# mitschabaude/montgomery

Hardware: AMD Instinct MI355X
Metric: BLS12-377 G1 MSM throughput (higher is better)
Workload: dtype u32

## Files before the change

### montgomery_amd/csrc/msm_sort.hip

```cpp
#include "msm_internal.h"

using namespace msm;
using namespace msmi;

namespace msmi {

uint64_t one_level_entry_limit(bool te) { return te ? 1ull << 22 : 1ull << 21; }

void sort_kernel_attributes() {
  HIPCHK(hipFuncSetAttribute((const void*)k_hist, hipFuncAttributeMaxDynamicSharedMemorySize, 128 * 1024));
  HIPCHK(hipFuncSetAttribute((const void*)k_scatter_lds, hipFuncAttributeMaxDynamicSharedMemorySize, 128 * 1024));
  HIPCHK(hipFuncSetAttribute((const void*)k_bin_split, hipFuncAttributeMaxDynamicSharedMemorySize, (int)bin_split_lds(1u << BS_MAX_AB)));
  HIPCHK(hipFuncSetAttribute((const void*)k_bin_pairs, hipFuncAttributeMaxDynamicSharedMemorySize, (int)bin_pairs_lds(1u << BS_MAX_FB)));
  HIPCHK(hipFuncSetAttribute((const void*)k_bin_slots, hipFuncAttributeMaxDynamicSharedMemorySize, (int)bin_slots_lds(1u << BS_MAX_FB)));
  const int dig_lds = 16 * (1 << BS_MAX_AB) * 4;
#define MSM_DIGITS_ATTR(ID, CV) HIPCHK(hipFuncSetAttribute((const void*)k_digits<CV>, hipFuncAttributeMaxDynamicSharedMemorySize, dig_lds));
  MSM_W_CURVES(MSM_DIGITS_ATTR)
#undef MSM_DIGITS_ATTR
  HIPCHK(hipFuncSetAttribute((const void*)te::k_te_digits, hipFuncAttributeMaxDynamicSharedMemorySize, dig_lds));
#define MSM_NARROW_ATTR(W)                                                                                                    \
  HIPCHK(hipFuncSetAttribute((const void*)k_digits_narrow<W>, hipFuncAttributeMaxDynamicSharedMemorySize, dig_lds));          \
  HIPCHK(hipFuncSetAttribute((const void*)k_te_digits_narrow<W>, hipFuncAttributeMaxDynamicSharedMemorySize, dig_lds));
  MSM_NARROW_WIDTHS(MSM_NARROW_ATTR)
#undef MSM_NARROW_ATTR
}

static void narrow_digits(msm_ctx* ctx, msm_ctx::Workspace& w, const uint32_t* d_scalars, uint64_t n, const Plan& pl, int k_lo, int kc_d,
                          bool bin_split, bool radix, uint32_t sortB, uint64_t pps, uint32_t hb, const WinSplit& ws) {
  hipStream_t s = w.stream;
  const bool te = ctx->is_te();
  const int W = pl.nar.width, per_lane = W == 1 ? 4 : W == 2 ? 2 : 1;
  uint32_t* dig = (uint32_t*)w.dig.p;
  uint32_t* err = (uint32_t*)ctx->errflag.p;
  const int fold = pl.fold ? 1 : 0;
  if (pl.batch) {
    if (bin_split || radix || k_lo != 0 || kc_d != pl.batch * pl.K || !pl.nar.nb) throw MsmFail{MSM_ERR_INTERNAL, "a batch group outside the one-level sort"};
    const uint32_t grid = (uint32_t)(((n + per_lane - 1) / per_lane + 255) / 256);
#define MSM_NARROW_LAUNCH_B(WW)                                                                                               \
  if (W == WW) {                                                                                                              \
    if (te) hipLaunchKernelGGL(k_te_digits_narrow_batch<WW>, dim3(grid), dim3(256), 0, s, dig, *pl.nar.nb, (uint32_t)pl.batch, \
                               (uint32_t)n, pl.c, pl.K, fold, pl.nar.fmt, err);                                               \
    else hipLaunchKernelGGL(k_digits_narrow_batch<WW>, dim3(grid), dim3(256), 0, s, dig, *pl.nar.nb, (uint32_t)pl.batch,      \
                            (uint32_t)n, pl.c, pl.K, fold, pl.nar.fmt, err);                                                  \
  }
    MSM_NARROW_WIDTHS(MSM_NARROW_LAUNCH_B)
#undef MSM_NARROW_LAUNCH_B
    return;
  }
  const uint32_t per = bin_split ? (uint32_t)pps : 256u * per_lane;
  const uint32_t grid = bin_split ? sortB : (uint32_t)((n + per - 1) / per);
  const uint32_t threads = bin_split ? 1024u : 256u;
  uint32_t* hist = bin_split ? (uint32_t*)w.block_hist.p : nullptr;
  const size_t lds = bin_split ? (size_t)kc_d * hb * 4 : 0;
  const uint64_t fbp = pack_fine_bits(ws);
#define MSM_NARROW_LAUNCH(WW)                                                                                                 \
  if (W == WW) {                                                                                                              \
    if (te) hipLaunchKernelGGL(k_te_digits_narrow<WW>, dim3(grid), dim3(threads), lds, s, dig, (const void*)d_scalars,        \
                               pl.nar.first, (uint32_t)n, pl.c, pl.K, k_lo, kc_d, fold, pl.nar.fmt, err, per, hist, hb, fbp); \
    else hipLaunchKernelGGL(k_digits_narrow<WW>, dim3(grid), dim3(threads), lds, s, dig, (const void*)d_scalars, pl.nar.first, \
                            (uint32_t)n, pl.c, pl.K, k_lo, kc_d, fold, pl.nar.fmt, err, per, hist, hb, fbp);                  \
  }
  MSM_NARROW_WIDTHS(MSM_NARROW_LAUNCH)
#undef MSM_NARROW_LAUNCH
}

void sort_window_group(msm_ctx* ctx, msm_ctx::Workspace& w, const uint32_t* d_scalars, uint64_t n, const Plan& pl, int k_lo, int k_hi,
                       GroupStats& st, SortOut& so, GroupDigits* share) {
  hipStream_t s = w.stream;
  const bool produce = share && share->produce;
  const bool consume = share && !share->produce && share->valid;
  const int kc_d = k_hi - k_lo;
  const uint32_t L = pl.L;
  const bool te = ctx->is_te();
  const uint64_t two_n_d = te ? n : 2 * n;
  const uint64_t n_entries = (uint64_t)kc_d * two_n_d;
  const int kc = pl.tables ? 1 : kc_d;
  const uint64_t two_n = pl.tables ? n_entries : two_n_d;
  const uint64_t nb = (uint64_t)kc * L;

  uint64_t mean = std::max<uint64_t>(1, two_n / (pl.fold ? L / 2 : L));
  uint64_t per_bucket_left = mean >= 512 ? 32 : (mean >= 128 || (mean >= 64 && pl.c >= 18 && !pl.tables)) ? 16 : 8;
  MSM_KNOB(per_bucket_left, "MSM_PBL", 1);
  uint32_t logG = 1;
  while (logG < 10 && (1ull << (logG + 1)) * per_bucket_left <= mean) logG++;

  if (!consume && !produce) ctx->ensure(w.dig, n_entries * 4);
  if (produce) {
    share->valid = false;
  } else {
  ctx->ensure(w.counts, nb * 4);
  ctx->ensure(w.cursor, (nb + 1) * 4);
  ctx->ensure(w.tail_off, (size_t)34 * (nb + 1) * 4);
  ctx->ensure(w.info, 64 * 4);
  }

  const int cbits = pl.L_log;
  const bool fits_lds = (size_t)L * 4 <= 128 * 1024;
  const bool want_radix = fits_lds && cbits > (int)RX_FINE_BITS && two_n >= one_level_entry_limit(te);
  const bool want_bins = !fits_lds || (pl.tables && two_n >= (1ull << 22));
  const bool bin_split = !fits_lds || want_bins;
  const bool radix = !bin_split && want_radix && cbits > (int)RX_FINE_BITS && cbits - (int)RX_FINE_BITS <= 8;
  WinSplit ws{};
  uint32_t hb = 1, nbmax = 1;
  if (bin_split) {
    if (kc > 16) throw MsmFail{MSM_ERR_INTERNAL, "more than 16 windows in a group of a window size above 16"};
    for (int kk = 0; kk < kc; kk++) {
      const bool top = (k_lo + kk) % pl.K == pl.K - 1;
      const int eff = pl.tables ? cbits : std::max(1, top ? std::min(cbits, pl.bits - (k_lo + kk) * pl.c) : std::min(cbits, pl.c - 1));
      const int ab_big = 10;
      const int abk = eff <= (int)ab_big ? eff : std::max((int)ab_big, eff - (int)BS_MAX_FB);
      if (abk > (int)BS_MAX_AB) throw MsmFail{MSM_ERR_INTERNAL, "window too wide for the bin split"};
      ws.ab[kk] = (uint8_t)abk;
      ws.fb[kk] = (uint8_t)(eff - abk);
      hb = std::max(hb, 1u << abk);
      nbmax = std::max(nbmax, 1u << (eff - abk));
    }
  } else if (radix) {
    if (kc > 16) throw MsmFail{MSM_ERR_INTERNAL, "more than 16 windows in a radix-split group"};
    for (int kk = 0; kk < kc; kk++) { ws.ab[kk] = (uint8_t)(cbits - (int)RX_FINE_BITS); ws.fb[kk] = (uint8_t)RX_FINE_BITS; }
  }
  const uint32_t Hn = radix ? 1u << (cbits - (int)RX_FINE_BITS) : 1u;
  const uint32_t V = (uint32_t)kc * (bin_split ? hb : Hn);
  uint32_t sortB = 1;
  uint64_t chunk = two_n, pps = n;
  if (bin_split) {
    const uint64_t mult = 4;
    sortB = (uint32_t)std::max<uint64_t>(1, std::min<uint64_t>((uint64_t)mult * ctx->n_cu, n / 4096));
    const uint64_t max_pps = (1ull << BS_SPAN_LOG) / (te ? 1 : 2);
    sortB = (uint32_t)std::max<uint64_t>(sortB, (n + max_pps - 1) / max_pps);
    pps = (n + sortB - 1) / sortB;
    chunk = (te ? 1 : 2) * pps;
    if (consume) {
      if (share->sortB != sortB || share->pps != pps || share->chunk != chunk || share->hb < hb)
        throw MsmFail{MSM_ERR_INTERNAL, "shared digits do not match the group's sort geometry"};
      hb = share->hb;
    } else {
      ctx->ensure(w.block_hist, (size_t)kc_d * sortB * hb * 4 + 64);
    }
  } else {
    const uint64_t mult = two_n >= (1ull << 27) ? 8 : two_n >= (1ull << 24) ? 4 : 2;
    uint64_t want = std::max<uint64_t>(1, (mult * ctx->n_cu + kc - 1) / kc);
    uint64_t maxb = std::max<uint64_t>(1, two_n / 8192);
    sortB = (uint32_t)std::min<uint64_t>(want, maxb);
    chunk = (two_n + sortB - 1) / sortB;
    if (!produce) ctx->ensure(w.block_hist, (size_t)kc * sortB * L * 4 + 64);
  }
  uint32_t* d_bin_start = nullptr;
  uint32_t *d_extra_first = nullptr, *d_mp_first = nullptr, *d_part_pair_off = nullptr;
  uint32_t part_len = 0, part_grid = 0;
  bool will_chunk = false;
  {
    const int chunk_rows_log = 23;
    const uint64_t table_rows = pl.tables ? (uint64_t)kc_d * n : n;
    const bool want_chunks = bin_split && !te && pl.c >= 18 && table_rows > (1ull << chunk_rows_log);
    will_chunk = bin_split && want_chunks && !te && logG >= 2;
  }
  if (produce && !bin_split) return;
  if (produce) ctx->ensure(w.dig, n_entries * 4);
  if (share && !share->produce && !bin_split) throw MsmFail{MSM_ERR_INTERNAL, "shared digits for a group that does not take the bin split"};
  const uint32_t* dig_p = consume ? share->dig + (uint64_t)(k_lo - share->k_lo) * two_n_d : (const uint32_t*)w.dig.p;
  uint32_t* hist_p = consume ? share->hist + (uint64_t)(k_lo - share->k_lo) * sortB * hb : (uint32_t*)w.block_hist.p;

  if (consume) HIPCHK(hipStreamWaitEvent(s, share->ready, 0));
  HIPCHK(hipEventRecord(w.ev[0], s));
  if (pl.nar.width) {
    if (!consume) narrow_digits(ctx, w, d_scalars, n, pl, k_lo, kc_d, bin_split, radix, sortB, pps, hb, ws);
  } else if (pl.batch) {
    if (bin_split || radix || k_lo != 0 || kc_d != pl.batch * pl.K) throw MsmFail{MSM_ERR_INTERNAL, "a batch group outside the one-level sort"};
    const uint32_t grid = (uint32_t)((n + 255) / 256);
    if (te)
      hipLaunchKernelGGL(te::k_te_digits_batch, dim3(grid), dim3(256), 0, s, (uint32_t*)w.dig.p, pl.batch_sc, (uint32_t)pl.batch,
                         (uint32_t)n, pl.c, pl.K, pl.strict ? 1 : 0, (uint32_t*)ctx->errflag.p);
    else
      W_LAUNCH(ctx, k_digits_batch, dim3(grid), dim3(256), 0, s, (uint32_t*)w.dig.p, pl.batch_sc, (uint32_t)pl.batch, (uint32_t)n, pl.c,
               pl.K, (pl.no_glv ? 0 : 1) | (pl.fold ? 2 : 0), pl.strict ? 1 : 0, (uint32_t*)ctx->errflag.p);
  } else if (!consume) {
    const uint32_t grid = bin_split ? sortB : (uint32_t)((n + 255) / 256);
    const uint32_t per = bin_split ? (uint32_t)pps : 256u;
    uint32_t* hist = bin_split ? (uint32_t*)w.block_hist.p : nullptr;
    const size_t lds = bin_split ? (size_t)kc_d * hb * 4 : 0;
    WinSplit ws_d = ws;
    if (pl.tables) for (int kk = 0; kk < 16; kk++) ws_d.fb[kk] = ws.fb[0];
    const uint32_t threads = bin_split ? 1024u : 256u;
    if (te)
      hipLaunchKernelGGL(te::k_te_digits, dim3(grid), dim3(threads), lds, s, (uint32_t*)w.dig.p, d_scalars, (uint32_t)n, pl.c, pl.K,
                         k_lo, kc_d, pl.strict ? 1 : 0, (uint32_t*)ctx->errflag.p, per, hist, hb, pack_fine_bits(ws_d), pl.b_lo, pl.b_n, pl.bt_lo, pl.bt_n);
    else
      W_LAUNCH(ctx, k_digits, dim3(grid), dim3(threads), lds, s, (uint32_t*)w.dig.p, d_scalars, (uint32_t)n, pl.c, pl.K, k_lo, kc_d,
                         (pl.no_glv ? 0 : 1) | (pl.fold ? 2 : 0), pl.strict ? 1 : 0, (uint32_t*)ctx->errflag.p, per, hist, hb, pack_fine_bits(ws_d), pl.b_lo, pl.b_n, pl.bt_lo, pl.bt_n);
  }
  if (produce) {
    share->k_lo = k_lo;
    share->dig = (const uint32_t*)w.dig.p;
    share->hist = (uint32_t*)w.block_hist.p;
    share->hb = hb;
    share->sortB = sortB;
    share->pps = pps;
    share->chunk = chunk;
    HIPCHK(hipEventRecord(share->ready, s));
    share->valid = true;
    return;
  }
  HIPCHK(hipEventRecord(w.ev[1], s));
  if (!bin_split) {
    hipLaunchKernelGGL(k_hist, dim3(sortB, kc), dim3(SORT_THREADS), (size_t)L * 4, s, (uint32_t*)w.block_hist.p,
                       (const uint32_t*)w.dig.p, two_n, chunk, L);
    hipLaunchKernelGGL(k_colscan, dim3((uint32_t)((nb + 255) / 256)), dim3(256), 0, s, (uint32_t*)w.block_hist.p,
                       (uint32_t*)w.counts.p, sortB, L, (uint32_t)kc);
  } else {
    ctx->ensure(w.part, ((size_t)2 * V + 2) * 4);
    uint32_t* d_bin_tot = (uint32_t*)w.part.p;
    d_bin_start = d_bin_tot + V;
    ctx->ensure(w.rec, n_entries * 8);
    hipLaunchKernelGGL(k_slice_scan, dim3((hb + 31) / 32, kc), dim3(1024), 0, s, hist_p, d_bin_tot,
                       pl.tables ? sortB * (uint32_t)kc_d : sortB, hb, (uint32_t)kc);
    part_len = (uint32_t)std::max<uint64_t>(1u << 16, ((2 * n_entries / V + BP_TILE - 1) / BP_TILE) * BP_TILE);
    part_grid = V + V / 2 + 1;
    ctx->ensure(w.parts, ((size_t)2 * (V + 1) + (V + 2)) * 4);
    d_extra_first = (uint32_t*)w.parts.p;
    d_mp_first = d_extra_first + (V + 1);
    d_part_pair_off = d_mp_first + (V + 1);
    PartTables ptab{d_extra_first, d_mp_first, d_part_pair_off, hb, part_len, {}};
    for (int kk = 0; kk < 16; kk++) ptab.fb[kk] = ws.fb[kk];
    hipLaunchKernelGGL(k_vscan, dim3(1), dim3(SCAN_THREADS), 0, s, d_bin_start, (const uint32_t*)d_bin_tot, V, (uint32_t*)w.info.p, ptab);
    const uint32_t per_block = (uint32_t)std::min<uint64_t>(std::min<uint64_t>(sortB, std::max<uint64_t>(1, (1ull << BS_SPAN_LOG) / chunk)),
                                                            std::max<uint64_t>(1, (2 * (uint64_t)BS_TILE + chunk - 1) / chunk));
    hipLaunchKernelGGL(k_bin_split, dim3((sortB + per_block - 1) / per_block, kc_d), dim3(BS_THREADS), bin_split_lds(hb), s, (uint2*)w.rec.p,
                       (const uint32_t*)d_bin_start, (const uint32_t*)hist_p, dig_p, two_n_d, chunk, hb, ws,
                       pl.tables ? 1u : 0u, sortB, per_block);
    bool spans_all = true;
    for (int kk = 0; kk < kc; kk++) spans_all &= (1u << ws.ab[kk]) == hb && (int)ws.ab[kk] + (int)ws.fb[kk] == cbits;
    if (!spans_all) HIPCHK(hipMemsetAsync(w.counts.p, 0, nb * 4, s));
    ctx->ensure(w.sub, (size_t)(V + 2) * nbmax * 4);
    hipLaunchKernelGGL(k_bin_count, dim3(part_grid), dim3(BC_THREADS), (size_t)nbmax * 4, s, (uint32_t*)w.counts.p, (const uint32_t*)d_bin_start,
                       (const uint2*)w.rec.p, hb, L, ws, (uint32_t*)w.info.p, V, (const uint32_t*)d_extra_first, (const uint32_t*)d_mp_first,
                       part_len, (uint32_t*)w.sub.p, nbmax);
    hipLaunchKernelGGL(k_part_scan, dim3(V), dim3(PSC_THREADS), 0, s, (uint32_t*)w.counts.p, (uint32_t*)w.sub.p, d_part_pair_off,
                       (const uint32_t*)d_extra_first, (const uint32_t*)d_mp_first, hb, L, nbmax, ws, (uint32_t*)w.info.p,
                       will_chunk ? 1u : 0u);
  }
  int RT = 0;
  uint64_t total_slots = 0;
  uint32_t max_bucket = 0;
  {
    if (!bin_split) {
      HIPCHK(hipMemsetAsync(w.info.p, 0, 64 * 4, s));
// ... 100 lines not shown
```

### montgomery_amd/csrc/msm_tree.hip

```cpp
#include "msm_internal.h"

using namespace msm;
using namespace msmi;

namespace msmi {

void accumulate_window_group(msm_ctx* ctx, msm_ctx::Workspace& w, const Plan& pl, int kc, uint64_t row_off, const SortOut& so,
                             GroupStats& st, TreeOut& to) {
  hipStream_t s = w.stream;
  const bool lone = pl.lone;
  const bool te = ctx->is_te();
  const uint32_t L = pl.L;
  const uint64_t nb = (uint64_t)kc * L;
  const size_t elem_bytes = te ? 128 : 96;
  const uint32_t logG = so.logG;
  const int RT = so.RT;
  const uint64_t total_slots = so.total_slots;
  const uint32_t max_bucket = so.max_bucket;
  const uint32_t* round1_slots = so.round1_slots;
  const uint32_t* round1_dest = so.round1_dest;
  const uint64_t rec_y_off = so.rec_y_off;
  const bool chunked = so.chunked;

  uint32_t FINISH_MAX = pl.c >= 18 ? 64 : 32;
  MSM_KNOB(FINISH_MAX, "MSM_FINISH_MAX", 1);
  uint32_t tail_min_pairs = pl.c >= 18 ? 1u << 23 : 1u << 21;
  MSM_KNOB(tail_min_pairs, "MSM_TAIL_MIN", 1);
  const bool use_finish = true;
  int r_stop = RT;
  if (use_finish) {
    uint32_t cap_elems = (max_bucket + (1u << logG) - 1) >> logG;
    r_stop = 0;
    while (r_stop < RT &&
           (((cap_elems + (1u << r_stop) - 1) >> r_stop) > FINISH_MAX || w.h_info[3 + r_stop + 1] >= tail_min_pairs))
      r_stop++;
  }
  uint64_t capA = 1, capB = 1;
  {
    int which = 0;
    uint64_t cnt = total_slots;
    for (uint32_t r = 1; r <= logG; r++) {
      cnt /= 2;
      if (r == 1 && chunked) continue;
      (which ? capB : capA) = std::max<uint64_t>(which ? capB : capA, cnt);
      which ^= 1;
    }
    for (int r = 1; r <= r_stop; r++) {
      cnt = w.h_info[3 + r];
      (which ? capB : capA) = std::max<uint64_t>(which ? capB : capA, cnt);
      which ^= 1;
    }
  }
  const size_t tree_slack = (size_t)2 * 257 * 512 * 16 + 4096;
  ctx->ensure(w.bufA, capA * elem_bytes + tree_slack);
  ctx->ensure(w.bufB, capB * elem_bytes + tree_slack);
  uint4* buf[2] = {(uint4*)w.bufA.p, (uint4*)w.bufB.p};
  uint64_t cap[2] = {capA, capB};
  int cur = 0;
  uint64_t n_in = total_slots;
  int round = 0;
  const uint4* fin = buf[0];
  uint64_t fin_cap = cap[0];
  const uint32_t* off_fin = (const uint32_t*)w.tail_off.p;
  if (total_slots > 0) {
    for (uint32_t r = 1; r <= logG; r++) {
      uint64_t n_out = n_in / 2;
      RoundGeom g = round_geom(ctx, n_out, r == 1 || (r == 2 && chunked) || te, lone);
      const uint64_t sstride = g.T;
      if (!te) ctx->ensure(w.scratch, (size_t)g.steps * NL * sstride * 4);
      BatchArgs a{};
      a.points = (pl.tables ? pl.tab_rows : (const uint32_t*)ctx->pts().rows.p) + row_off * ctx->row_words();
      a.slots = r == 1 ? round1_slots : (const uint32_t*)w.slots.p;
      a.dest = r == 1 ? round1_dest : nullptr;
      a.in = buf[cur ^ 1];
      a.in_cap = cap[cur ^ 1];
      a.out = buf[cur];
      a.out_cap = cap[cur];
      a.scratch = (uint32_t*)w.scratch.p;
      a.sstride = sstride;
      a.n_out = n_out;
      a.steps = g.steps;
      const bool rows_out = r == 1 && chunked, rows_in = r == 2 && chunked;
      a.y_off = 4 * ctx->nw();
      if (rows_out) a.out_rows = (uint32_t*)w.rows1.p;
      if (rows_in) { a.points = (const uint32_t*)w.rows1.p; a.slots = nullptr; }
      if (rows_out) a.out_y_off = rec_y_off;
      if (rows_in && ctx->nw() == 12) a.y_off = rec_y_off;
      if (r == 1 || rows_in) {
        if (te) hipLaunchKernelGGL(te::k_te_add<MODE_GATHER>, dim3(g.grid), dim3(256), 0, s, a);
        else W_LAUNCH_MODE(ctx, k_batch_add, MODE_GATHER, dim3(g.grid), dim3(256), 0, s, a);
        if (r == 1) HIPCHK(hipEventRecord(w.ev[6], s));
      } else {
        if (te) hipLaunchKernelGGL(te::k_te_add<MODE_REGULAR>, dim3(g.grid), dim3(256), 0, s, a);
        else W_LAUNCH_MODE(ctx, k_batch_add, MODE_REGULAR, dim3(g.grid), dim3(256), 0, s, a);
      }
      st.n_pairs += n_out;
      n_in = n_out;
      round++;
      if (rows_out) continue;
      fin = buf[cur];
      fin_cap = cap[cur];
      cur ^= 1;
    }
    for (int r = 1; r <= r_stop; r++) {
      uint64_t n_out = w.h_info[3 + r];
      RoundGeom g = round_geom(ctx, n_out, te);
      const uint64_t sstride = g.T;
      if (!te) ctx->ensure(w.scratch, (size_t)g.steps * NL * sstride * 4);
      BatchArgs a{};
      a.in = buf[cur ^ 1];
      a.in_cap = cap[cur ^ 1];
      a.out = buf[cur];
      a.out_cap = cap[cur];
      a.scratch = (uint32_t*)w.scratch.p;
      a.sstride = sstride;
      a.n_out = n_out;
      a.steps = g.steps;
      if (n_out) {
        const uint32_t* off_in = (const uint32_t*)w.tail_off.p + (uint64_t)(r - 1) * (nb + 1);
        const uint32_t* off_out = (const uint32_t*)w.tail_off.p + (uint64_t)r * (nb + 1);
        ctx->ensure(w.desc, n_out * 4);
        hipLaunchKernelGGL(k_tail_desc, dim3((uint32_t)((n_out + 255) / 256)), dim3(256), 0, s, (uint32_t*)w.desc.p, off_in,
                           off_out, (uint32_t)nb, (uint32_t)n_out);
        a.desc = (const uint32_t*)w.desc.p;
        if (te) hipLaunchKernelGGL(te::k_te_add<MODE_SEARCH>, dim3(g.grid), dim3(256), 0, s, a);
        else W_LAUNCH_MODE(ctx, k_batch_add, MODE_SEARCH, dim3(g.grid), dim3(256), 0, s, a);
      }
      st.n_pairs += n_out;
      fin = buf[cur];
      fin_cap = cap[cur];
      cur ^= 1;
      round++;
    }
    off_fin = (const uint32_t*)w.tail_off.p + (uint64_t)r_stop * (nb + 1);
  }
  st.rounds += round;
  const uint32_t* bucket_proj = nullptr;
  if (use_finish && total_slots > 0) {
    ctx->ensure(w.bucket_proj, nb * (te ? 4 * te::TL : 3 * NL) * 4);
    const uint32_t* perm = nullptr;
    if (nb >= 4096) {
      ctx->ensure(w.blk_tab2, (nb + 2 * FINISH_BINS) * 4);
      uint32_t* hist = (uint32_t*)w.blk_tab2.p;
      HIPCHK(hipMemsetAsync(hist, 0, 2 * FINISH_BINS * 4, s));
      const uint32_t fgrid = (uint32_t)((nb + FINISH_THREADS - 1) / FINISH_THREADS);
      hipLaunchKernelGGL(k_finish_hist, dim3(fgrid), dim3(FINISH_THREADS), 0, s, off_fin, (uint32_t)nb, hist);
      hipLaunchKernelGGL(k_finish_perm, dim3(fgrid), dim3(FINISH_THREADS), 0, s, off_fin, (uint32_t)nb,
                         (const uint32_t*)hist, hist + FINISH_BINS, hist + 2 * FINISH_BINS);
      perm = hist + 2 * FINISH_BINS;
    }
    if (te)
      hipLaunchKernelGGL(te::k_te_bucket_finish, dim3((uint32_t)((nb + 255) / 256)), dim3(256), 0, s, (uint32_t*)w.bucket_proj.p,
                         fin, fin_cap, off_fin, (uint32_t)nb, perm);
    else
      W_LAUNCH(ctx, k_bucket_finish, dim3((uint32_t)((nb + 255) / 256)), dim3(256), 0, s, (uint32_t*)w.bucket_proj.p, fin,
                         fin_cap, off_fin, (uint32_t)nb, perm);
    bucket_proj = (const uint32_t*)w.bucket_proj.p;
  }
  if (total_slots == 0) HIPCHK(hipEventRecord(w.ev[6], s));
  HIPCHK(hipEventRecord(w.ev[3], s));
  to.fin = fin;
  to.fin_cap = fin_cap;
  to.off_fin = off_fin;
  to.bucket_proj = bucket_proj;
}

}
```

### montgomery_amd/csrc/sort_kernels.h

```cpp
#pragma once
#include "msm_kernels.h"

namespace msm {


constexpr int SCAN_THREADS = 1024;
constexpr int SCAN_ITEMS = 4;

__device__ __forceinline__ void lds_barrier() {
#if defined(__HIP_DEVICE_COMPILE__)
  asm volatile("s_waitcnt lgkmcnt(0)\n\ts_barrier" ::: "memory");
#endif
}

template <bool LDS_ONLY = false>
MSM_DEV uint32_t block_excl_scan(uint32_t v, uint32_t* lds_wave, uint32_t& total) {
  uint32_t x = v;
  const int lane = threadIdx.x & 63, wave = threadIdx.x >> 6;
#pragma unroll
  for (int d = 1; d < 64; d <<= 1) {
    uint32_t y = __shfl_up(x, d, 64);
    if (lane >= d) x += y;
  }
  if (LDS_ONLY) lds_barrier(); else __syncthreads();
  if (lane == 63) lds_wave[wave] = x;
  if (LDS_ONLY) lds_barrier(); else __syncthreads();
  uint32_t wave_base = 0, tot = 0;
  const int nw = blockDim.x >> 6;
  for (int w = 0; w < nw; w++) {
    uint32_t t = lds_wave[w];
    if (w < wave) wave_base += t;
    tot += t;
  }
  total = tot;
  return wave_base + x - v;
}


constexpr int PS_BLOCK = 1024;
constexpr int PS_ITEMS = 4;
constexpr int PS_SPAN = PS_BLOCK * PS_ITEMS;

MSM_DEV uint32_t scan_quantity(uint32_t n, uint32_t logG, int q) {
  const uint32_t cg = (n + ((1u << logG) - 1)) >> logG;
  if (q == 0) return cg << logG;
  const int r = q - 1;
  return (cg + ((1u << r) - 1)) >> r;
}

constexpr int PS_MAX_NQ = 34;
MSM_DEV int pscan_nq(const uint32_t* info, uint32_t logG) {
  const uint32_t capmax = (info[1] + ((1u << logG) - 1)) >> logG;
  int rt = 0;
  while (rt < 32 && (1u << rt) < capmax) rt++;
  return rt + 2;
}

constexpr int INFO_ALGO_PAIRS = 40;
__global__ void __launch_bounds__(256) k_bucket_max(const uint32_t* counts, uint32_t nb, uint32_t* info)
#ifndef MSM_SORT_TU
    ;
#else
{
  __shared__ uint32_t lds_max;
  __shared__ unsigned long long lds_sum;
  if (threadIdx.x == 0) { lds_max = 0; lds_sum = 0; }
  __syncthreads();
  uint32_t mx = 0;
  unsigned long long sum = 0;
  for (uint32_t b = blockIdx.x * blockDim.x + threadIdx.x; b < nb; b += gridDim.x * blockDim.x) {
    const uint32_t cnt = counts[b];
    mx = max(mx, cnt);
    sum += cnt ? cnt - 1 : 0;
  }
  for (int o = 32; o > 0; o >>= 1) sum += __shfl_down(sum, o);
  atomicMax(&lds_max, mx);
  if ((threadIdx.x & 63) == 0) atomicAdd(&lds_sum, sum);
  __syncthreads();
  if (threadIdx.x == 0) {
    atomicMax(&info[1], lds_max);
    atomicAdd(reinterpret_cast<unsigned long long*>(info + INFO_ALGO_PAIRS), lds_sum);
  }
}
#endif

__global__ void __launch_bounds__(PS_BLOCK) k_pscan_partial(const uint32_t* counts, uint32_t nb, uint32_t logG, const uint32_t* info,
                                                            uint32_t* partial, uint32_t nblocks)
#ifndef MSM_SORT_TU
    ;
#else
{
  __shared__ uint32_t lds_wave[PS_BLOCK / 64];
  const int nq = pscan_nq(info, logG);
  const uint32_t b0 = blockIdx.x * PS_SPAN + threadIdx.x * PS_ITEMS;
  uint32_t n[PS_ITEMS];
#pragma unroll
  for (int j = 0; j < PS_ITEMS; j++) n[j] = (b0 + j) < nb ? counts[b0 + j] : 0u;
  for (int q = 0; q < nq; q++) {
    uint32_t sum = 0;
#pragma unroll
    for (int j = 0; j < PS_ITEMS; j++) sum += scan_quantity(n[j], logG, q);
    uint32_t tot;
    block_excl_scan(sum, lds_wave, tot);
    if (threadIdx.x == 0) partial[(uint64_t)q * nblocks + blockIdx.x] = tot;
  }
}
#endif

__global__ void __launch_bounds__(SCAN_THREADS) k_pscan_top(uint32_t* partial, uint32_t nblocks, uint32_t logG, uint32_t* info)
#ifndef MSM_SORT_TU
    ;
#else
{
  __shared__ uint32_t lds_wave[SCAN_THREADS / 64];
  const int nq = pscan_nq(info, logG);
  for (int q = 0; q < nq; q++) {
    uint32_t* p = partial + (uint64_t)q * nblocks;
    uint32_t carry = 0;
    for (uint32_t base = 0; base < nblocks; base += SCAN_THREADS) {
      uint32_t i = base + threadIdx.x;
      uint32_t v = i < nblocks ? p[i] : 0u;
      uint32_t tot;
      uint32_t ex = block_excl_scan(v, lds_wave, tot) + carry;
      if (i < nblocks) p[i] = ex;
      carry += tot;
    }
    if (threadIdx.x == 0) {
      if (q == 0) info[0] = carry; else info[3 + (q - 1)] = carry;
    }
  }
}
#endif

__global__ void __launch_bounds__(PS_BLOCK) k_pscan_final(const uint32_t* counts, uint32_t nb, uint32_t logG,
                                                          const uint32_t* partial, uint32_t nblocks, uint32_t* cursor,
                                                          uint32_t* tail_off, const uint32_t* info)
#ifndef MSM_SORT_TU
    ;
#else
{
  __shared__ uint32_t lds_wave[PS_BLOCK / 64];
  const int nq = pscan_nq(info, logG);
  const uint32_t b0 = blockIdx.x * PS_SPAN + threadIdx.x * PS_ITEMS;
  uint32_t n[PS_ITEMS];
#pragma unroll
  for (int j = 0; j < PS_ITEMS; j++) n[j] = (b0 + j) < nb ? counts[b0 + j] : 0u;
  for (int q = 0; q < nq; q++) {
    uint32_t v[PS_ITEMS], sum = 0;
#pragma unroll
    for (int j = 0; j < PS_ITEMS; j++) { v[j] = scan_quantity(n[j], logG, q); sum += v[j]; }
    uint32_t tot;
    uint32_t ex = block_excl_scan(sum, lds_wave, tot) + partial[(uint64_t)q * nblocks + blockIdx.x];
    uint32_t* out = q == 0 ? cursor : tail_off + (uint64_t)(q - 1) * (nb + 1);
#pragma unroll
    for (int j = 0; j < PS_ITEMS; j++) {
      if (b0 + j < nb) out[b0 + j] = ex;
      ex += v[j];
    }
    if (blockIdx.x == 0 && threadIdx.x == 0) out[nb] = q == 0 ? info[0] : info[3 + (q - 1)];
  }
}
#endif


constexpr int SORT_THREADS = 1024;



__device__ __forceinline__ uint32_t lds_rank_add(uint32_t* lds, uint32_t bin, bool valid) {
  const uint32_t first = __builtin_amdgcn_readfirstlane(bin);
  const uint64_t same = __ballot(valid && bin == first);
  if (__popcll(same) >= 16) {
    const uint32_t lane = threadIdx.x & 63u;
    const int leader = __ffsll((long long)same) - 1;
    uint32_t base = 0;
    if ((int)lane == leader) base = atomicAdd(&lds[first], (uint32_t)__popcll(same));
    base = __shfl(base, leader, 64);
    const uint32_t r = base + (uint32_t)__popcll(same & ((1ull << lane) - 1ull));
    if ((same >> lane) & 1ull) return r;
    return valid ? atomicAdd(&lds[bin], 1u) : 0u;
  }
  return valid ? atomicAdd(&lds[bin], 1u) : 0u;
}

__global__ void __launch_bounds__(SORT_THREADS) k_hist(uint32_t* block_hist, const uint32_t* dig, uint64_t two_n,
                                                       uint64_t chunk, uint32_t L)
#ifndef MSM_SORT_TU
    ;
#else
{
  extern __shared__ uint32_t lds_hist[];
  const uint32_t b = blockIdx.x, kk = blockIdx.y, B = gridDim.x;
  constexpr uint32_t shift = 0;
  const uint64_t hist_row = (uint64_t)kk * B + b;
  for (uint32_t l = threadIdx.x; l < L; l += SORT_THREADS) lds_hist[l] = 0;
  __syncthreads();
  const uint64_t beg = (uint64_t)b * chunk, end = min(beg + chunk, two_n);
  const uint32_t* d = dig + (uint64_t)kk * two_n;
  uint64_t j0 = beg;
  if (end > beg) {
    const uint64_t head = min<uint64_t>(end - beg, (16u - (uint32_t)(reinterpret_cast<uintptr_t>(d + beg) & 15u)) % 16u / 4u);
    if (head) {
      const uint32_t l = threadIdx.x < head ? d[beg + threadIdx.x] & 0x7FFFFFFFu : 0u;
      (void)lds_rank_add(lds_hist, l ? (l - 1) >> shift : 0u, l != 0);
      j0 = beg + head;
    }
  }
  if (end > j0) {
    const uint4* dv = reinterpret_cast<const uint4*>(d + j0);
    const uint64_t nvec = (end - j0) / 4;
    for (uint64_t q0 = 0; q0 < nvec; q0 += 2 * SORT_THREADS) {
      const uint64_t qa = q0 + threadIdx.x, qb = qa + SORT_THREADS;
      const uint4 va = qa < nvec ? dv[qa] : make_uint4(0, 0, 0, 0);
      const uint4 vb = qb < nvec ? dv[qb] : make_uint4(0, 0, 0, 0);
      const uint32_t w[8] = {va.x, va.y, va.z, va.w, vb.x, vb.y, vb.z, vb.w};
#pragma unroll
      for (int i = 0; i < 8; i++) {
        const uint32_t l = w[i] & 0x7FFFFFFFu;
        (void)lds_rank_add(lds_hist, l ? (l - 1) >> shift : 0u, l != 0);
      }
    }
    j0 += nvec * 4;
  }
  for (; j0 < end; j0 += SORT_THREADS) {
    const uint64_t j = j0 + threadIdx.x;
    const uint32_t l = j < end ? d[j] & 0x7FFFFFFFu : 0u;
    (void)lds_rank_add(lds_hist, l ? (l - 1) >> shift : 0u, l != 0);
  }
  __syncthreads();
  uint32_t* out = block_hist + hist_row * L;
  for (uint32_t l = threadIdx.x; l < L; l += SORT_THREADS) out[l] = lds_hist[l];
}
#endif

__global__ void __launch_bounds__(256) k_colscan(uint32_t* block_hist, uint32_t* counts, uint32_t B, uint32_t L, uint32_t k_cnt)
#ifndef MSM_SORT_TU
    ;
#else
{
  uint64_t id = (uint64_t)blockIdx.x * blockDim.x + threadIdx.x;
  if (id >= (uint64_t)k_cnt * L) return;
  uint32_t kk = (uint32_t)(id / L), l = (uint32_t)(id - (uint64_t)kk * L);
  uint32_t* p = block_hist + (uint64_t)kk * B * L + l;
  uint32_t run = 0, b = 0;
  for (; b + 8 <= B; b += 8) {
    uint32_t v[8];
#pragma unroll
    for (int i = 0; i < 8; i++) v[i] = p[(uint64_t)(b + i) * L];
#pragma unroll
    for (int i = 0; i < 8; i++) { p[(uint64_t)(b + i) * L] = run; run += v[i]; }
  }
  for (; b < B; b++) {
    uint32_t v = p[(uint64_t)b * L];
    p[(uint64_t)b * L] = run;
    run += v;
  }
  counts[id] = run;
}
#endif

__global__ void __launch_bounds__(SORT_THREADS) k_scatter_lds(uint32_t* slots, const uint32_t* cursor,
                                                              const uint32_t* block_hist, const uint32_t* dig,
                                                              uint64_t two_n, uint64_t chunk, uint32_t L)
#ifndef MSM_SORT_TU
    ;
#else
{
// ... 759 lines not shown
```

### montgomery_amd/csrc/tree_kernels.h

```cpp
#pragma once
#include "msm_kernels.h"

namespace msm {


__global__ void __launch_bounds__(256) k_tail_desc(uint32_t* desc, const uint32_t* off_in, const uint32_t* off_out, uint32_t nb,
                                                   uint32_t n_out)
#ifndef MSM_SORT_TU
    ;
#else
{
  __shared__ uint32_t run[2];
  const uint32_t e0 = blockIdx.x * blockDim.x;
  const uint32_t e = e0 + threadIdx.x;
  if (threadIdx.x == 0 || threadIdx.x == blockDim.x - 1) {
    const uint32_t ee = min(threadIdx.x == 0 ? e0 : e0 + blockDim.x - 1, n_out - 1);
    uint32_t lo = 0, hi = nb;
    while (hi - lo > 1) {
      const uint32_t mid = (lo + hi) >> 1;
      if (off_out[mid] <= ee) lo = mid; else hi = mid;
    }
    run[threadIdx.x == 0 ? 0 : 1] = lo;
  }
  __syncthreads();
  if (e >= n_out) return;
  uint32_t lo = run[0], hi = run[1] + 1;
  while (hi - lo > 1) {
    const uint32_t mid = (lo + hi) >> 1;
    if (off_out[mid] <= e) lo = mid; else hi = mid;
  }
  uint32_t j = e - off_out[lo];
  uint32_t ia = off_in[lo] + 2 * j;
  desc[e] = (ia << 1) | ((ia + 1) < off_in[lo + 1] ? 1u : 0u);
}
#endif

template <int W>
__global__ void __launch_bounds__(256) k_test_rows_to_planes(uint4* planes, uint64_t cap, const uint32_t* rows, uint32_t n) {
  uint32_t e = blockIdx.x * blockDim.x + threadIdx.x;
  if (e >= n) return;
  uint32_t w[W];
  load_words12(w, rows + (uint64_t)e * ROW_WORDS);
  store_planes3(planes, cap, 0, e, w);
  load_words12(w, rows + (uint64_t)e * ROW_WORDS + W);
  store_planes3(planes, cap, W / 4, e, w);
}


constexpr int FINISH_BINS = 64;

MSM_DEV uint32_t finish_bin(const uint32_t* off, uint32_t b) {
  uint32_t c = off[b + 1] - off[b];
  return c < FINISH_BINS ? c : FINISH_BINS - 1;
}

constexpr int FINISH_THREADS = 1024;

__global__ void __launch_bounds__(FINISH_THREADS) k_finish_hist(const uint32_t* off, uint32_t nb, uint32_t* hist)
#ifndef MSM_SORT_TU
    ;
#else
{
  __shared__ uint32_t lh[FINISH_BINS];
  if (threadIdx.x < FINISH_BINS) lh[threadIdx.x] = 0;
  __syncthreads();
  const uint32_t b = blockIdx.x * blockDim.x + threadIdx.x;
  if (b < nb) atomicAdd(&lh[finish_bin(off, b)], 1u);
  __syncthreads();
  if (threadIdx.x < FINISH_BINS && lh[threadIdx.x]) atomicAdd(&hist[threadIdx.x], lh[threadIdx.x]);
}
#endif

__global__ void __launch_bounds__(FINISH_THREADS) k_finish_perm(const uint32_t* off, uint32_t nb, const uint32_t* hist,
                                                                uint32_t* cursor, uint32_t* perm)
#ifndef MSM_SORT_TU
    ;
#else
{
  __shared__ uint32_t lcnt[FINISH_BINS], lbase[FINISH_BINS];
  if (threadIdx.x < FINISH_BINS) lcnt[threadIdx.x] = 0;
  __syncthreads();
  const uint32_t b = blockIdx.x * blockDim.x + threadIdx.x;
  const bool active = b < nb;
  const uint32_t key = active ? finish_bin(off, b) : 0u;
  uint32_t rank = 0;
  if (active) rank = atomicAdd(&lcnt[key], 1u);
  __syncthreads();
  if (threadIdx.x < FINISH_BINS && lcnt[threadIdx.x]) {
    uint32_t base = 0;
    for (uint32_t k = FINISH_BINS - 1; k > threadIdx.x; k--) base += hist[k];
    lbase[threadIdx.x] = base + atomicAdd(&cursor[threadIdx.x], lcnt[threadIdx.x]);
  }
  __syncthreads();
  if (active) perm[lbase[key] + rank] = b;
}
#endif

}
```

Baseline: 518.4 million.

## Build all tail-round descriptors and finish histogram in one batched kernel

```diff
diff --git a/montgomery_amd/csrc/msm_sort.hip b/montgomery_amd/csrc/msm_sort.hip
--- a/montgomery_amd/csrc/msm_sort.hip
+++ b/montgomery_amd/csrc/msm_sort.hip
@@ -91,7 +91,7 @@
   ctx->ensure(w.counts, nb * 4);
   ctx->ensure(w.cursor, (nb + 1) * 4);
   ctx->ensure(w.tail_off, (size_t)34 * (nb + 1) * 4);
-  ctx->ensure(w.info, 64 * 4);
+  ctx->ensure(w.info, INFO_WORDS * 4);
   }
 
   const int cbits = pl.L_log;
diff --git a/montgomery_amd/csrc/msm_tree.hip b/montgomery_amd/csrc/msm_tree.hip
--- a/montgomery_amd/csrc/msm_tree.hip
+++ b/montgomery_amd/csrc/msm_tree.hip
@@ -62,6 +62,7 @@
   const uint4* fin = buf[0];
   uint64_t fin_cap = cap[0];
   const uint32_t* off_fin = (const uint32_t*)w.tail_off.p;
+  uint32_t* finish_hist = nullptr;
   if (total_slots > 0) {
     for (uint32_t r = 1; r <= logG; r++) {
       uint64_t n_out = n_in / 2;
@@ -102,6 +103,22 @@
       fin_cap = cap[cur];
       cur ^= 1;
     }
+    uint64_t n_desc = 0;
+    for (int r = 1; r <= r_stop; r++) n_desc += w.h_info[3 + r];
+    finish_hist = use_finish && nb >= 4096 ? (uint32_t*)w.info.p + INFO_FINISH : nullptr;
+    if (n_desc || finish_hist) {
+      ctx->ensure(w.desc, std::max<uint64_t>(n_desc, 1) * 4);
+      const uint32_t cap_elems = (max_bucket + (1u << logG) - 1) >> logG;
+      uint32_t heavy_rounds = 0;
+      while ((int)heavy_rounds < r_stop && ((cap_elems + (2u << heavy_rounds) - 1) >> (heavy_rounds + 1)) >= TD_TILE) heavy_rounds++;
+      const uint32_t bucket_blocks = (uint32_t)((nb + TD_SPAN - 1) / TD_SPAN);
+      const uint64_t tile_outputs = (uint64_t)TD_TILE * (TD_THREADS / 64);
+      const uint32_t tile_blocks = heavy_rounds ? (uint32_t)((w.h_info[3 + 1] + tile_outputs - 1) / tile_outputs) : 0;
+      hipLaunchKernelGGL(k_tail_descs, dim3(bucket_blocks + tile_blocks, (uint32_t)r_stop + (finish_hist ? 1 : 0)), dim3(TD_THREADS), 0, s,
+                         (uint32_t*)w.desc.p, (const uint32_t*)w.tail_off.p, (uint32_t)nb, (uint32_t)r_stop, heavy_rounds,
+                         bucket_blocks, finish_hist);
+    }
+    const uint32_t* desc = (const uint32_t*)w.desc.p;
     for (int r = 1; r <= r_stop; r++) {
       uint64_t n_out = w.h_info[3 + r];
       RoundGeom g = round_geom(ctx, n_out, te);
@@ -117,12 +134,8 @@
       a.n_out = n_out;
       a.steps = g.steps;
       if (n_out) {
-        const uint32_t* off_in = (const uint32_t*)w.tail_off.p + (uint64_t)(r - 1) * (nb + 1);
-        const uint32_t* off_out = (const uint32_t*)w.tail_off.p + (uint64_t)r * (nb + 1);
-        ctx->ensure(w.desc, n_out * 4);
-        hipLaunchKernelGGL(k_tail_desc, dim3((uint32_t)((n_out + 255) / 256)), dim3(256), 0, s, (uint32_t*)w.desc.p, off_in,
-                           off_out, (uint32_t)nb, (uint32_t)n_out);
-        a.desc = (const uint32_t*)w.desc.p;
+        a.desc = desc;
+        desc += n_out;
         if (te) hipLaunchKernelGGL(te::k_te_add<MODE_SEARCH>, dim3(g.grid), dim3(256), 0, s, a);
         else W_LAUNCH_MODE(ctx, k_batch_add, MODE_SEARCH, dim3(g.grid), dim3(256), 0, s, a);
       }
@@ -139,15 +152,12 @@
   if (use_finish && total_slots > 0) {
     ctx->ensure(w.bucket_proj, nb * (te ? 4 * te::TL : 3 * NL) * 4);
     const uint32_t* perm = nullptr;
-    if (nb >= 4096) {
-      ctx->ensure(w.blk_tab2, (nb + 2 * FINISH_BINS) * 4);
-      uint32_t* hist = (uint32_t*)w.blk_tab2.p;
-      HIPCHK(hipMemsetAsync(hist, 0, 2 * FINISH_BINS * 4, s));
+    if (finish_hist) {
+      ctx->ensure(w.blk_tab2, nb * 4);
       const uint32_t fgrid = (uint32_t)((nb + FINISH_THREADS - 1) / FINISH_THREADS);
-      hipLaunchKernelGGL(k_finish_hist, dim3(fgrid), dim3(FINISH_THREADS), 0, s, off_fin, (uint32_t)nb, hist);
       hipLaunchKernelGGL(k_finish_perm, dim3(fgrid), dim3(FINISH_THREADS), 0, s, off_fin, (uint32_t)nb,
-                         (const uint32_t*)hist, hist + FINISH_BINS, hist + 2 * FINISH_BINS);
-      perm = hist + 2 * FINISH_BINS;
+                         (const uint32_t*)finish_hist, finish_hist + FINISH_BINS, (uint32_t*)w.blk_tab2.p);
+      perm = (const uint32_t*)w.blk_tab2.p;
     }
     if (te)
       hipLaunchKernelGGL(te::k_te_bucket_finish, dim3((uint32_t)((nb + 255) / 256)), dim3(256), 0, s, (uint32_t*)w.bucket_proj.p,
diff --git a/montgomery_amd/csrc/sort_kernels.h b/montgomery_amd/csrc/sort_kernels.h
--- a/montgomery_amd/csrc/sort_kernels.h
+++ b/montgomery_amd/csrc/sort_kernels.h
@@ -57,6 +57,7 @@
 }
 
 constexpr int INFO_ALGO_PAIRS = 40;
+constexpr int INFO_FINISH = 64, INFO_FINISH_WORDS = 128, INFO_WORDS = INFO_FINISH + INFO_FINISH_WORDS;
 __global__ void __launch_bounds__(256) k_bucket_max(const uint32_t* counts, uint32_t nb, uint32_t* info)
 #ifndef MSM_SORT_TU
     ;
@@ -113,6 +114,7 @@
 #else
 {
   __shared__ uint32_t lds_wave[SCAN_THREADS / 64];
+  if (threadIdx.x < INFO_FINISH_WORDS) info[INFO_FINISH + threadIdx.x] = 0;
   const int nq = pscan_nq(info, logG);
   for (int q = 0; q < nq; q++) {
     uint32_t* p = partial + (uint64_t)q * nblocks;
diff --git a/montgomery_amd/csrc/tree_kernels.h b/montgomery_amd/csrc/tree_kernels.h
--- a/montgomery_amd/csrc/tree_kernels.h
+++ b/montgomery_amd/csrc/tree_kernels.h
@@ -1,37 +1,107 @@
 #pragma once
-#include "msm_kernels.h"
+#include "sort_kernels.h"
 
 namespace msm {
 
 
-__global__ void __launch_bounds__(256) k_tail_desc(uint32_t* desc, const uint32_t* off_in, const uint32_t* off_out, uint32_t nb,
-                                                   uint32_t n_out)
+constexpr int FINISH_BINS = 64;
+static_assert(2 * FINISH_BINS == INFO_FINISH_WORDS, "k_pscan_top zeroes the histogram and the cursors of k_finish_perm");
+
+MSM_DEV uint32_t finish_bin(const uint32_t* off, uint32_t b) {
+  uint32_t c = off[b + 1] - off[b];
+  return c < FINISH_BINS ? c : FINISH_BINS - 1;
+}
+
+constexpr int TD_THREADS = 256;
+constexpr int TD_RUNS = 4;
+constexpr uint32_t TD_SPAN = TD_THREADS * TD_RUNS;
+constexpr uint32_t TD_TILE = 1024;
+
+__global__ void __launch_bounds__(TD_THREADS) k_tail_descs(uint32_t* desc, const uint32_t* tail_off, uint32_t nb, uint32_t r_stop,
+                                                           uint32_t heavy_rounds, uint32_t bucket_blocks, uint32_t* hist)
 #ifndef MSM_SORT_TU
     ;
 #else
 {
-  __shared__ uint32_t run[2];
-  const uint32_t e0 = blockIdx.x * blockDim.x;
-  const uint32_t e = e0 + threadIdx.x;
-  if (threadIdx.x == 0 || threadIdx.x == blockDim.x - 1) {
-    const uint32_t ee = min(threadIdx.x == 0 ? e0 : e0 + blockDim.x - 1, n_out - 1);
-    uint32_t lo = 0, hi = nb;
-    while (hi - lo > 1) {
-      const uint32_t mid = (lo + hi) >> 1;
-      if (off_out[mid] <= ee) lo = mid; else hi = mid;
+  const uint64_t row = (uint64_t)nb + 1;
+  if (blockIdx.y == r_stop) {
+    __shared__ uint32_t lh[FINISH_BINS];
+    if (threadIdx.x < FINISH_BINS) lh[threadIdx.x] = 0;
+    __syncthreads();
+    const uint32_t* off = tail_off + r_stop * row;
+#pragma unroll
+    for (int j = 0; j < TD_RUNS; j++) {
+      const uint32_t b = blockIdx.x * TD_SPAN + j * TD_THREADS + threadIdx.x;
+      if (b < nb) atomicAdd(&lh[finish_bin(off, b)], 1u);
     }
-    run[threadIdx.x == 0 ? 0 : 1] = lo;
+    __syncthreads();
+    if (threadIdx.x < FINISH_BINS && lh[threadIdx.x]) atomicAdd(&hist[threadIdx.x], lh[threadIdx.x]);
+    return;
   }
-  __syncthreads();
-  if (e >= n_out) return;
-  uint32_t lo = run[0], hi = run[1] + 1;
-  while (hi - lo > 1) {
-    const uint32_t mid = (lo + hi) >> 1;
-    if (off_out[mid] <= e) lo = mid; else hi = mid;
+  const uint32_t r = blockIdx.y + 1;
+  const uint32_t* off_in = tail_off + (r - 1) * row;
+  const uint32_t* off_out = tail_off + r * row;
+  uint64_t first = 0;
+  for (uint32_t q = 1; q < r; q++) first += tail_off[q * row + nb];
+  uint32_t* d = desc + first;
+  const uint32_t lane = threadIdx.x & 63u, wave = threadIdx.x >> 6;
+  if (blockIdx.x < bucket_blocks) {
+    for (int j = 0; j < TD_RUNS; j++) {
+      const uint32_t b0 = blockIdx.x * TD_SPAN + (wave * TD_RUNS + j) * 64;
+      if (b0 >= nb) break;
+      const uint32_t b = min(b0 + lane, nb), b1 = min(b + 1, nb);
+      const uint32_t o = off_out[b], in0 = off_in[b], in1 = off_in[b1];
+      const uint32_t cnt = off_out[b1] - o;
+      const uint32_t mine = cnt < TD_TILE ? cnt : 0u;
+      uint32_t start = mine;
+#pragma unroll
+      for (int s = 1; s < 64; s <<= 1) {
+        const uint32_t y = __shfl_up(start, s, 64);
+        if ((int)lane >= s) start += y;
+      }
+      const uint32_t total = __shfl(start, 63, 64);
+      start -= mine;
+      for (uint32_t i0 = 0; i0 < total; i0 += 64) {
+        const uint32_t i = i0 + lane;
+        uint32_t l = 0;
+#pragma unroll
+        for (int s = 32; s > 0; s >>= 1)
+          if (__shfl(start, l + s, 64) <= i) l += s;
+        const uint32_t k = i - __shfl(start, l, 64);
+        const uint32_t ia = __shfl(in0, l, 64) + 2 * k;
+        const uint32_t e = __shfl(o, l, 64) + k, end = __shfl(in1, l, 64);
+        if (i < total) d[e] = (ia << 1) | ((ia + 1) < end ? 1u : 0u);
+      }
+    }
+  } else {
+    if (r > heavy_rounds) return;
+    const uint32_t n_out = off_out[nb];
+    const uint64_t t0 = ((uint64_t)(blockIdx.x - bucket_blocks) * (TD_THREADS / 64) + wave) * TD_TILE;
+    if (t0 >= n_out) return;
+    const uint32_t t1 = (uint32_t)min<uint64_t>(t0 + TD_TILE, n_out);
+    uint32_t seen = 0xFFFFFFFFu;
+    for (int side = 0; side < 2; side++) {
+      const uint32_t e = side == 0 ? (uint32_t)t0 : t1 - 1;
+      uint32_t lo = 0, hi = nb;
+      while (hi - lo > 1) {
+        const uint32_t step = (hi - lo + 63) / 64;
+        const uint32_t p = lo + lane * step;
+        const bool le = p < hi && off_out[p] <= e;
+        lo += ((uint32_t)__popcll(__ballot(le)) - 1) * step;
+        hi = min(hi, lo + step);
+      }
+      if (lo == seen) break;
+      seen = lo;
+      const uint32_t o0 = off_out[lo], o1 = off_out[lo + 1];
+      if (o1 - o0 < TD_TILE) continue;
+      const uint32_t in0 = off_in[lo], in1 = off_in[lo + 1];
+      const uint32_t end = min(o1, t1);
+      for (uint32_t x = max(o0, (uint32_t)t0) + lane; x < end; x += 64) {
+        const uint32_t ia = in0 + 2 * (x - o0);
+        d[x] = (ia << 1) | ((ia + 1) < in1 ? 1u : 0u);
+      }
+    }
   }
-  uint32_t j = e - off_out[lo];
-  uint32_t ia = off_in[lo] + 2 * j;
-  desc[e] = (ia << 1) | ((ia + 1) < off_in[lo + 1] ? 1u : 0u);
 }
 #endif
 
@@ -47,29 +117,7 @@
 }
 
 
-constexpr int FINISH_BINS = 64;
-
-MSM_DEV uint32_t finish_bin(const uint32_t* off, uint32_t b) {
-  uint32_t c = off[b + 1] - off[b];
-  return c < FINISH_BINS ? c : FINISH_BINS - 1;
-}
-
 constexpr int FINISH_THREADS = 1024;
-
-__global__ void __launch_bounds__(FINISH_THREADS) k_finish_hist(const uint32_t* off, uint32_t nb, uint32_t* hist)
-#ifndef MSM_SORT_TU
-    ;
-#else
-{
-  __shared__ uint32_t lh[FINISH_BINS];
-  if (threadIdx.x < FINISH_BINS) lh[threadIdx.x] = 0;
-  __syncthreads();
-  const uint32_t b = blockIdx.x * blockDim.x + threadIdx.x;
-  if (b < nb) atomicAdd(&lh[finish_bin(off, b)], 1u);
-  __syncthreads();
-  if (threadIdx.x < FINISH_BINS && lh[threadIdx.x]) atomicAdd(&hist[threadIdx.x], lh[threadIdx.x]);
-}
-#endif
 
 __global__ void __launch_bounds__(FINISH_THREADS) k_finish_perm(const uint32_t* off, uint32_t nb, const uint32_t* hist,
                                                                 uint32_t* cursor, uint32_t* perm)
```

Result: no change. 518.0 million (-0.1%).
